# jgrodzki/radix_sort

Hardware: AMD Instinct MI355X
Metric: Gkeys/sec (u64) (higher is better)
Workload: dtype u64

## Files before the change

radix_sort_amd/csrc/rsx_launch_impl.hpp:

```cpp
#pragma once
#include <cstdlib>
#include "rsx_internal.hpp"
#include "rsx_small_kernel.hpp"
#include "rsx_mid_kernels.hpp"
#include "rsx_segment_kernels.hpp"
#include "rsx_segment_pairs_kernels.hpp"

#ifndef RSX_HIST_BLOCKS_PER_CU
#define RSX_HIST_BLOCKS_PER_CU 8
#endif

namespace rsxh {

inline uint32_t rank_atomic_of(const rsx_ctx* ctx) { return (ctx->rank_atomic && !(ctx->options & OPT_BALLOT_RANKS)) ? 1u : 0u; }
constexpr CleanList CLEAN_NONE = {{nullptr, nullptr, nullptr}, {0, 0, 0}};

inline uint64_t hist_blocks_per_region(const rsx_ctx* ctx, const RegionGeom& g) {
    const uint64_t per_block = 512ull * 16;
    uint64_t bpr = ((1ull << g.region_shift) + per_block - 1) / per_block;
    const uint64_t cap = ((uint64_t)ctx->num_cu * RSX_HIST_BLOCKS_PER_CU + g.num_regions - 1) / g.num_regions;
    if (bpr > cap) bpr = cap;
    return bpr == 0 ? 1 : bpr;
}
template <int ES, bool FLT>
// ... 354 lines not shown
    if (grid < parts) grid = parts;
    LaunchTimer lt(ctx, RSX_PROF_HIST, st);
    hipLaunchKernelGGL(rsx_marginal16_kernel<ES>, dim3(grid), dim3(256), 0, st, P, parts, k, g, J, jclear, status32(g) ? 1u : 0u,
                       static_cast<uint4*>(ctx->status), zero16_n, run.clean, run.gate);
    RSX_HIP(hipGetLastError());
    run.clean = CLEAN_NONE;
    return RSX_OK;
}

template <int ES>
int launch_bucket16(rsx_ctx* ctx, const SortRun& run, void* data, void* scratch, size_t n, const rsx_layout* L, const uint64_t* starts,
                    const WidePlan* plan, hipStream_t st) {
    if constexpr (ES < 4) {
        return fail(ctx, RSX_ERR_INTERNAL, "launch_bucket16: narrow elements");
    } else {
        constexpr int KPT = bucket_kpt_for(ES);
        if (L->key_bytes < 4) return fail(ctx, RSX_ERR_INTERNAL, "launch_bucket16: key width out of range");
        SmallArgs a = small_args(ctx, L, L->key_bytes - 2, L->key_bytes, false);
        a.src = data;
        a.data = data;
        a.cap = bucket_cap(ES);
        LaunchTimer lt(ctx, RSX_PROF_OTHER, st);
        const uint64_t avg = (uint64_t)n / 65536u;
        const uint32_t gs = group_shift(ctx, n, L);
        const Gate base = run.gate;
        auto go = [&](auto wgc, auto kc, uint32_t form, uint32_t group_shift) {
            constexpr int WGS = decltype(wgc)::value;
            constexpr int K = decltype(kc)::value;
            SmallArgs b = a;
            b.group_shift = group_shift;
            if (group_shift) b.passes = L->key_bytes;
            static_assert(cape<ES, K, WGS>() == bucket_cape(ES, K, WGS), "host and device agree on what a workgroup holds");
            const size_t lds = (size_t)cape<ES, K, WGS>() * ES + (WGS / 64) * RADIX * bucket_cnt_bytes() + 64 + 3 * RADIX * sizeof(uint32_t);
            auto kern = rsx_bucket16_kernel<ES, K, WGS>;
            ensure_lds(ctx, reinterpret_cast<const void*>(kern), lds);
            int per_cu = (int)((size_t)163840 / lds);
            if (per_cu < 1) per_cu = 1;
            if (per_cu > 4 * RSX_B16_WAVES(WGS) * 64 / WGS) per_cu = 4 * RSX_B16_WAVES(WGS) * 64 / WGS;
            const Gate g{base.word, VERDICT_PATH_MASK | VERDICT_FORM_MASK, VERDICT_HYBRID | form};
            hipLaunchKernelGGL(kern, dim3((uint32_t)(ctx->num_cu * per_cu)), dim3(WGS), lds, st, b, starts, scratch, plan, g);
        };
        using std::integral_constant;
        constexpr int KBIG = wide_kpt_for(ES);
        if (gs >= 2) go(integral_constant<int, 512>{}, integral_constant<int, KPT>{}, VERDICT_GROUPS, gs);
        if (avg <= (uint64_t)256 * KPT) go(integral_constant<int, 256>{}, integral_constant<int, KPT>{}, VERDICT_WG256, 0);
        if (avg <= (uint64_t)512 * KPT) go(integral_constant<int, 512>{}, integral_constant<int, KPT>{}, VERDICT_WG512, 0);
        const bool big_form = KBIG != KPT && wide_big_form(ES, n);
        if (big_form) go(integral_constant<int, 1024>{}, integral_constant<int, KBIG>{}, VERDICT_WG1024, 0);
        else go(integral_constant<int, 1024>{}, integral_constant<int, KPT>{}, VERDICT_WG1024, 0);
        {
            constexpr int KMED = medium_kpt_for(ES);
            const size_t lds = (size_t)cape<ES, KMED, 1024>() * ES + 16 * RADIX * bucket_cnt_bytes() + 64 + 3 * RADIX * sizeof(uint32_t);
            auto kern = rsx_bucket16_medium_kernel<ES, KMED, 1024>;
            ensure_lds(ctx, reinterpret_cast<const void*>(kern), lds);
            const Gate g{base.word, VERDICT_PATH_MASK | VERDICT_MEDIUM, VERDICT_HYBRID | VERDICT_MEDIUM};
            hipLaunchKernelGGL(kern, dim3((uint32_t)ctx->num_cu), dim3(1024), lds, st, a, starts, scratch, plan, (uint32_t)(256 * KPT), (uint32_t)(512 * KPT),
                               (uint32_t)(big_form ? cape<ES, KBIG, 1024>() : cape<ES, KPT, 1024>()), g);
        }
        RSX_HIP(hipGetLastError());
        return RSX_OK;
    }
}

template <int ES>
int launch_segcopy(rsx_ctx* ctx, const void* src, void* dst, const uint64_t* so, const uint64_t* dof,
                   const uint64_t* len, uint32_t nseg, hipStream_t st) {
    const uint32_t bps = 8;
// ... 162 lines not shown
```

radix_sort_amd/csrc/rsx_small_kernel.hpp:

```cpp
#pragma once
#include "rsx_device.hpp"

namespace rsx {

struct SmallArgs {
    const void* src;
    void* data;
    uint32_t n;
    uint32_t passes;
    uint32_t rank_atomic;
    uint32_t map_load;
    uint32_t map_store;
    DigitSpec spec[16];
    KeyXform xf;
    const uint32_t* top_tot;
    uint32_t cap;
    uint32_t no_skip;
    uint32_t group_shift;
    uint32_t key_offset, key_bytes;
    uint32_t* hint;
};

struct PassPlan {
    uint32_t first, end;
    uint32_t mask[8];
    uint32_t low[8];
    __device__ __forceinline__ void set_masks(const uint32_t key_offset, const uint32_t key_bytes) {
#pragma unroll
        for (int w = 0; w < 8; ++w) {
            uint32_t m = 0, l = 0;
#pragma unroll
            for (uint32_t b = 0; b < 4; ++b) {
                const uint32_t byte = 4u * (uint32_t)w + b;
                if (byte >= key_offset + first && byte < key_offset + key_bytes) m |= 0xFFu << (8u * b);
                if (byte >= key_offset && byte < key_offset + first) l |= 0xFFu << (8u * b);
            }
            mask[w] = m;
            low[w] = l;
        }
    }
};

#ifndef RSX_MEND_SLACK
#define RSX_MEND_SLACK 6u
#endif
__device__ __forceinline__ uint32_t first_digit_for(const uint32_t m, const uint32_t variable_bits, const uint32_t end) {
    const uint32_t lg = m <= 1u ? 0u : 32u - (uint32_t)__builtin_clz(m - 1u);
    const uint32_t need = 2u * lg > RSX_MEND_SLACK ? 2u * lg - RSX_MEND_SLACK : 0u;
    uint32_t first = variable_bits > need ? (variable_bits - need) >> 3 : 0u;
    if (first + 1u > end) first = end != 0u ? end - 1u : 0u;
    return first;
}

template <int ES>
struct WaveCnt {
    static constexpr bool HALF = false;
    using T = typename std::conditional<HALF, uint16_t, uint32_t>::type;
    static __device__ __forceinline__ void zero(T* my, uint32_t lane) {
        uint32_t* w = reinterpret_cast<uint32_t*>(my);
#pragma unroll
        for (int i = 0; i < (HALF ? 2 : 4); ++i) w[i * WAVE + lane] = 0;
    }
    static __device__ __forceinline__ uint32_t add_rtn(T* my, uint32_t d, uint32_t v) {
        if constexpr (HALF) {
            const uint32_t sh = (d & 1u) * 16u;
            return (atomicAdd(reinterpret_cast<uint32_t*>(my) + (d >> 1), v << sh) >> sh) & 0xFFFFu;
        } else {
            return atomicAdd(&my[d], v);
        }
    }
};
template <int ES, int KPT, int WG>
__host__ __device__ constexpr uint32_t cape() {
    constexpr uint32_t slots = (uint32_t)WG * KPT;
    constexpr uint32_t room = ((163840u - 1024u - (uint32_t)(WG / WAVE) * RADIX * (uint32_t)sizeof(typename WaveCnt<ES>::T) - 64u - 3u * RADIX * 4u) / (uint32_t)ES) & ~3u;
    return slots < room ? slots : room;
}

template <int ES, int KPT, int WG>
__device__ __forceinline__ void local_load(const SmallArgs& a, const Elem<ES>* __restrict__ src, const uint32_t n, Elem<ES> (&e)[KPT]) {
    const uint32_t tid = threadIdx.x, lane = tid & 63u, wave = tid >> 6;
    const uint32_t kp = (n + WG - 1) / WG;
    const uint32_t seg = wave * (WAVE * kp) + lane;
#pragma unroll
    for (int j = 0; j < KPT; ++j) {
        e[j] = Elem<ES>{};
        if ((uint32_t)j < kp) {
            const uint32_t p = seg + (uint32_t)j * WAVE;
            if (p < n) {
                e[j] = src[p];
                if (a.map_load) key_map<ES, false>(e[j], a.xf);
            }
        }
    }
}

template <int ES, int KPT, int WG>
__device__ __forceinline__ void local_passes(const SmallArgs& a, Elem<ES> (&e)[KPT], const uint32_t n, unsigned char* smem,
                                             const uint32_t first = 0, const uint32_t end = ~0u) {
    const uint32_t stop = end == ~0u ? a.passes : end;
    constexpr int NWAVE = WG / WAVE;
    using E = Elem<ES>;
    E* s_elems = reinterpret_cast<E*>(smem);
    using C = WaveCnt<ES>;
    typename C::T* s_cnt = reinterpret_cast<typename C::T*>(smem + (size_t)cape<ES, KPT, WG>() * sizeof(E));
    uint32_t* s_misc = reinterpret_cast<uint32_t*>(s_cnt + NWAVE * RADIX);
    const uint32_t tid = threadIdx.x, lane = tid & 63u, wave = tid >> 6;
    const uint32_t kp = (n + WG - 1) / WG;
    const uint32_t seg = wave * (WAVE * kp) + lane;
    typename C::T* my = s_cnt + wave * RADIX;
    for (uint32_t pass = first; pass < stop; ++pass) {
        const DigitSpec spec = a.spec[pass];
        C::zero(my, lane);
        auto digit_of = [&](int j) -> uint32_t {
            return (seg + (uint32_t)j * WAVE >= n) ? 255u : elem_digit<ES, false>(e[j], spec);
        };
        uint32_t rk[KPT];
#pragma unroll
        for (int j = 0; j < KPT; ++j) {
            rk[j] = 0;
            if ((uint32_t)j < kp) {
                const uint32_t d = digit_of(j);
                if (a.rank_atomic) {
                    rk[j] = C::add_rtn(my, d, 1u);
                } else {
                    const uint64_t m = match_digit(d);
                    const uint32_t below = mbcnt64(m);
                    const uint32_t seen = my[d];
                    if (below == 0) (void)C::add_rtn(my, d, (uint32_t)__popcll(m));
                    rk[j] = seen + below;
                }
            }
        }
        __syncthreads();
        uint32_t tcount = 0, incl = 0;
        if (tid < RADIX) {
#pragma unroll
            for (int w = 0; w < NWAVE; ++w) tcount += s_cnt[w * RADIX + tid];
            incl = wave_incl_scan<true>(tcount);
            if (lane == 63) s_misc[wave] = incl;
        }
        __syncthreads();
        if (tid < RADIX) {
            uint32_t run = incl - tcount;
            for (uint32_t w = 0; w < wave; ++w) run += s_misc[w];
#pragma unroll
            for (int w = 0; w < NWAVE; ++w) {
                const uint32_t c = s_cnt[w * RADIX + tid];
                s_cnt[w * RADIX + tid] = (typename C::T)run;
                run += c;
            }
        }
        __syncthreads();
#pragma unroll
        for (int j = 0; j < KPT; ++j)
            if ((uint32_t)j < kp) {
                if constexpr (cape<ES, KPT, WG>() < (uint32_t)WG * KPT) {
                    if (seg + (uint32_t)j * WAVE < n) s_elems[(uint32_t)my[digit_of(j)] + rk[j]] = e[j];
                } else {
                    s_elems[(uint32_t)my[digit_of(j)] + rk[j]] = e[j];
                }
            }
        __syncthreads();
        if (pass + 1 < stop) {
#pragma unroll
            for (int j = 0; j < KPT; ++j)
                if ((uint32_t)j < kp) e[j] = s_elems[seg + (uint32_t)j * WAVE];
        }
    }
}

template <int ES, int KPT, int WG>
__device__ __forceinline__ void local_store(const SmallArgs& a, Elem<ES>* __restrict__ dst, const uint32_t n, unsigned char* smem) {
    const Elem<ES>* s_elems = reinterpret_cast<const Elem<ES>*>(smem);
    for (uint32_t i = threadIdx.x; i < n; i += WG) {
        Elem<ES> x = s_elems[i];
        if (a.map_store) key_map<ES, true>(x, a.xf);
        dst[i] = x;
    }
}

template <int ES, int KPT, int WG>
__device__ __forceinline__ void local_sort(const SmallArgs& a, const Elem<ES>* __restrict__ src, Elem<ES>* __restrict__ dst,
                                           const uint32_t n, unsigned char* smem) {
    Elem<ES> e[KPT];
    local_load<ES, KPT, WG>(a, src, n, e);
    local_passes<ES, KPT, WG>(a, e, n, smem);
    local_store<ES, KPT, WG>(a, dst, n, smem);
}

template <int ES, int KPT, int WG, typename DigitFn>
__device__ __forceinline__ void stream_pass(const SmallArgs& a, const Elem<ES>* __restrict__ src, Elem<ES>* __restrict__ dst, const uint32_t m,
                                            unsigned char* smem, DigitFn digit, const bool map_back, uint32_t& bin_start, uint32_t& bin_count) {
    constexpr int NWAVE = WG / WAVE;
    constexpr uint32_t CH = cape<ES, KPT, WG>();
    using E = Elem<ES>;
    E* s_elems = reinterpret_cast<E*>(smem);
    using C = WaveCnt<ES>;
    typename C::T* s_cnt = reinterpret_cast<typename C::T*>(smem + (size_t)cape<ES, KPT, WG>() * sizeof(E));
    uint32_t* s_misc = reinterpret_cast<uint32_t*>(s_cnt + NWAVE * RADIX);
    uint32_t* s_gbase = s_misc + NWAVE;
    uint32_t* s_dstart = s_gbase + RADIX;
// ... 100 lines not shown
    using E = Elem<ES>;
    E* src = buf0;
    E* dst = buf1;
    for (uint32_t pass = 0; pass < a.passes; ++pass) {
        const DigitSpec spec = a.spec[pass];
        uint32_t bs = 0, bc = 0;
        stream_pass<ES, KPT, WG>(a, src, dst, m, smem, [&](const E& x) { return elem_digit<ES, false>(x, spec); },
                                 pass + 1 == a.passes && a.map_store != 0, bs, bc);
        E* t = src;
        src = dst;
        dst = t;
    }
}

#define RSX_B16_WAVES(WG) ((WG) >= 512 ? 4 : 3)
template <int ES>
__device__ __forceinline__ bool agree(const PassPlan& pp, const Elem<ES>& x, const Elem<ES>& y) {
    uint32_t diff = 0;
#pragma unroll
    for (int w = 0; w < ES / 4; ++w) diff |= (x.w[w] ^ y.w[w]) & pp.mask[w];
    return diff == 0;
}
constexpr uint32_t MEND_LIST = 192;
template <int ES, int KPT, int WG>
__device__ __forceinline__ uint32_t* mend_count(unsigned char* smem) {
    return reinterpret_cast<uint32_t*>(smem + (size_t)cape<ES, KPT, WG>() * sizeof(Elem<ES>));
}
template <int ES, int KPT, int WG>
__device__ __forceinline__ bool local_check(const PassPlan& pp, const uint32_t n, unsigned char* smem, Elem<ES> (&x)[KPT], uint32_t& ties) {
    using E = Elem<ES>;
    const E* s_elems = reinterpret_cast<const E*>(smem);
    ties = 0;
    if (threadIdx.x == 0) *mend_count<ES, KPT, WG>(smem) = 0;
#pragma unroll
    for (int j = 0; j < KPT; ++j) {
        const uint32_t i = (uint32_t)j * WG + threadIdx.x;
        x[j] = E{};
        if (i < n) {
            x[j] = s_elems[i];
            const E p = s_elems[i != 0 ? i - 1 : 0];
            uint32_t diff = 0;
#pragma unroll
            for (int w = 0; w < ES / 4; ++w) diff |= (x[j].w[w] ^ p.w[w]) & pp.mask[w];
            ties |= (diff == 0 && i != 0) ? 1u << j : 0u;
        }
    }
    uint32_t work = 0;
    for (uint32_t t = ties; t != 0; t &= t - 1u) {
        const uint32_t i = (uint32_t)__builtin_ctz(t) * WG + threadIdx.x;
        const E u = s_elems[i], v = s_elems[i - 1];
#pragma unroll
        for (int w = 0; w < ES / 4; ++w) work |= (u.w[w] ^ v.w[w]) & pp.low[w];
    }
    return __syncthreads_or(work != 0 ? 1 : 0) != 0;
}
#ifndef RSX_MEND_INLINE
#define RSX_MEND_INLINE __forceinline__
#endif
template <int ES>
struct MendMasks {
    uint32_t hi[ES / 4], lo[ES / 4];
};
template <int ES>
__device__ RSX_MEND_INLINE uint32_t mend_listed(Elem<ES>* s_elems, uint32_t* s_list, uint32_t* s_flag, const uint32_t n, const uint32_t wg,
                                                          uint32_t ties, const MendMasks<ES> mm) {
    using E = Elem<ES>;
    constexpr uint32_t MAX_RUN = 48;
    auto same = [&](const E& u, const E& v) {
        uint32_t diff = 0;
#pragma unroll
        for (int w = 0; w < ES / 4; ++w) diff |= (u.w[w] ^ v.w[w]) & mm.hi[w];
        return diff == 0;
    };
    auto less = [&](const E& u, const E& v) {
#pragma unroll
        for (int w = ES / 4 - 1; w >= 0; --w) {
            const uint32_t a = u.w[w] & mm.lo[w], b = v.w[w] & mm.lo[w];
// ... 16 lines not shown
        const uint32_t i = s_list[1 + threadIdx.x];
        uint32_t len = 2;
        while (i + len < n && len <= MAX_RUN && same(s_elems[i + len], s_elems[i])) ++len;
        if (len > MAX_RUN) {
            *s_flag = 1;
        } else {
            for (uint32_t k = 1; k < len; ++k) {
                const E y = s_elems[i + k];
                uint32_t j = k;
                while (j > 0 && less(y, s_elems[i + j - 1])) {
                    s_elems[i + j] = s_elems[i + j - 1];
                    --j;
                }
                s_elems[i + j] = y;
            }
        }
    }
    __syncthreads();
    return *s_flag == 0 ? 1u : 0u;
}
template <int ES, int KPT, int WG>
__device__ __forceinline__ bool local_mend_listed(const uint32_t n, unsigned char* smem, const PassPlan& pp, uint32_t* s_flag, const uint32_t ties) {
    static_assert((WG / WAVE) * RADIX >= MEND_LIST + 1, "the list lives in the wave counters");
    MendMasks<ES> mm;
#pragma unroll
    for (int w = 0; w < ES / 4; ++w) {
        mm.hi[w] = pp.mask[w];
        mm.lo[w] = pp.low[w];
    }
    return mend_listed<ES>(reinterpret_cast<Elem<ES>*>(smem), mend_count<ES, KPT, WG>(smem), s_flag, n, (uint32_t)WG, ties, mm) != 0;
}
template <int ES, int KPT, int WG>
__device__ __forceinline__ void local_store_regs(const SmallArgs& a, Elem<ES>* __restrict__ dst, const uint32_t n, Elem<ES> (&x)[KPT]) {
#pragma unroll
    for (int j = 0; j < KPT; ++j) {
        const uint32_t i = (uint32_t)j * WG + threadIdx.x;
        if (i < n) {
            if (a.map_store) key_map<ES, true>(x[j], a.xf);
            dst[i] = x[j];
        }
    }
}

template <int ES, int KPT, int WG>
__device__ __forceinline__ bool local_finish(const SmallArgs& a, Elem<ES>* __restrict__ dst, const uint32_t n, unsigned char* smem, const PassPlan& pp,
                                             uint32_t* s_flag) {
    Elem<ES> x[KPT];
    uint32_t ties;
    if (!local_check<ES, KPT, WG>(pp, n, smem, x, ties)) {
        local_store_regs<ES, KPT, WG>(a, dst, n, x);
        return true;
    }
    if (!local_mend_listed<ES, KPT, WG>(n, smem, pp, s_flag, ties)) return false;
    local_store<ES, KPT, WG>(a, dst, n, smem);
    return true;
}

template <int ES, int KPT, int WG>
__device__ __forceinline__ void local_sort_skip(const SmallArgs& a, const Elem<ES>* __restrict__ src, Elem<ES>* __restrict__ dst, const uint32_t n,
                                                unsigned char* smem, PassPlan& pp, uint32_t* s_flag) {
    using E = Elem<ES>;
    E e[KPT];
    local_load<ES, KPT, WG>(a, src, n, e);
    local_passes<ES, KPT, WG>(a, e, n, smem, pp.first, pp.end);
    if (pp.first == 0) {
        local_store<ES, KPT, WG>(a, dst, n, smem);
    } else if (!local_finish<ES, KPT, WG>(a, dst, n, smem, pp, s_flag)) {
        pp.first = 0;
        const uint32_t kp = (n + WG - 1) / WG, seg = (threadIdx.x >> 6) * (WAVE * kp) + (threadIdx.x & 63u);
#pragma unroll
        for (int j = 0; j < KPT; ++j)
            if ((uint32_t)j < kp) e[j] = reinterpret_cast<const E*>(smem)[seg + (uint32_t)j * WAVE];
        __syncthreads();
        local_passes<ES, KPT, WG>(a, e, n, smem, 0, pp.end);
        local_store<ES, KPT, WG>(a, dst, n, smem);
    }
}

template <int ES, int KPT>
__global__ __launch_bounds__(512) void rsx_small_sort_kernel(const SmallArgs a) {
    extern __shared__ __attribute__((aligned(16))) unsigned char smem[];
    local_sort<ES, KPT, 512>(a, static_cast<const Elem<ES>*>(a.src), static_cast<Elem<ES>*>(a.data), a.n, smem);
}

template <int ES, int KPT, int WG>
__global__ __launch_bounds__(WG) void rsx_bucket_sort_kernel(const SmallArgs a) {
    extern __shared__ __attribute__((aligned(16))) unsigned char smem[];
    uint64_t* s_red = reinterpret_cast<uint64_t*>(smem);
    const uint32_t tid = threadIdx.x, v = blockIdx.x;
    uint64_t c = 0;
    if (tid < RADIX) {
        c = a.top_tot[tid];
        if (tid == v) s_red[4] = c;
        if (v == 0) {
            uint64_t big = c;
#pragma unroll
            for (int o = 32; o > 0; o >>= 1) {
                const uint64_t y = __shfl_xor(big, o);
                big = y > big ? y : big;
            }
            if ((tid & 63u) == 0u) s_red[5 + (tid >> 6)] = big;
        }
        uint64_t below = tid < v ? c : 0ull;
#pragma unroll
        for (int o = 32; o > 0; o >>= 1) below += __shfl_xor(below, o);
        if ((tid & 63u) == 0u) s_red[tid >> 6] = below;
    }
    __syncthreads();
    const uint64_t start = s_red[0] + s_red[1] + s_red[2] + s_red[3];
    const uint64_t count = s_red[4];
    if (v == 0 && tid == 0) {
        uint64_t big = s_red[5];
        for (int w = 1; w < 4; ++w) big = s_red[5 + w] > big ? s_red[5 + w] : big;
        __hip_atomic_store(a.hint, big <= (uint64_t)a.cap / 4 ? 1u : big <= (uint64_t)a.cap ? 3u : 2u, __ATOMIC_RELAXED, __HIP_MEMORY_SCOPE_SYSTEM);
    }
    __syncthreads();
    if (count == 0) return;
    if (count > (uint64_t)cape<ES, KPT, WG>()) {
        big_bucket_sort<ES, KPT, WG>(a, const_cast<Elem<ES>*>(static_cast<const Elem<ES>*>(a.src)) + start,
                                     static_cast<Elem<ES>*>(a.data) + start, (uint32_t)count, smem);
        return;
    }
    if constexpr (ES < 8) {
        local_sort<ES, KPT, WG>(a, static_cast<const Elem<ES>*>(a.src) + start, static_cast<Elem<ES>*>(a.data) + start, (uint32_t)count, smem);
    } else {
        PassPlan pp;
        pp.end = a.passes;
        pp.first = a.no_skip ? 0u : first_digit_for((uint32_t)count, 8u * a.passes, a.passes);
        pp.set_masks(a.key_offset, a.key_bytes);
        uint32_t* s_flag = reinterpret_cast<uint32_t*>(reinterpret_cast<typename WaveCnt<ES>::T*>(smem + (size_t)cape<ES, KPT, WG>() * sizeof(Elem<ES>)) + (WG / WAVE) * RADIX) + (WG / WAVE);
        local_sort_skip<ES, KPT, WG>(a, static_cast<const Elem<ES>*>(a.src) + start, static_cast<Elem<ES>*>(a.data) + start, (uint32_t)count, smem, pp,
                                     s_flag);
    }
}

template <int ES, int KPT, int WG>
__global__ __launch_bounds__(WG, RSX_B16_WAVES(WG)) void rsx_bucket16_kernel(const SmallArgs a, const uint64_t* __restrict__ starts, void* scratch,
                                                                         const WidePlan* __restrict__ plan, Gate gate) {
    extern __shared__ __attribute__((aligned(16))) unsigned char smem[];
    if (!gate_open(gate)) return;
    using E = Elem<ES>;
    constexpr int NWAVE = WG / WAVE;
    uint32_t* s_flag = reinterpret_cast<uint32_t*>(reinterpret_cast<typename WaveCnt<ES>::T*>(smem + (size_t)cape<ES, KPT, WG>() * sizeof(E)) + NWAVE * RADIX) + NWAVE;
    const uint32_t gs = a.group_shift != 0 ? plan->group_shift : 0;
    const bool medium = (plan->verdict & VERDICT_MEDIUM) != 0;
    PassPlan pp;
    pp.end = gs == 0 ? plan->pass_end : plan->group_end;
    if (pp.end == 0) {
        if (a.map_store) {
            const uint64_t n = starts[65536];
            E* data = static_cast<E*>(a.data);
            for (uint64_t i = (uint64_t)blockIdx.x * WG + threadIdx.x; i < n; i += (uint64_t)gridDim.x * WG) {
                E x = data[i];
                key_map<ES, true>(x, a.xf);
                data[i] = x;
            }
        }
        return;
    }
    const uint32_t b_lo = plan->window_top - 15u;
    const uint32_t end_sub = pp.end;
    if (gs != 0) pp.end = (b_lo + gs + 7u) / 8u;
    {
        const uint64_t big = (uint64_t)plan->scan_max << gs;
        const uint32_t m = big < (uint64_t)cape<ES, KPT, WG>() ? (uint32_t)big : cape<ES, KPT, WG>();
        pp.first = a.no_skip ? 0u : first_digit_for(m, b_lo + gs, pp.end);
    }
    pp.set_masks(a.key_offset, a.key_bytes);
    for (uint32_t g = blockIdx.x; g < (65536u >> gs); g += gridDim.x) {
        const uint32_t b0 = g << gs;
        const uint64_t gstart = starts[b0];
        const uint64_t gcount = starts[b0 + (1u << gs)] - gstart;
        if (gcount == 0) continue;
        const bool whole = gs == 0 || gcount <= (uint64_t)cape<ES, KPT, WG>();
        const uint32_t nsub = whole ? 1u : 1u << gs;
        for (uint32_t sub = 0; sub < nsub; ++sub) {
            uint64_t start = gstart, count = gcount;
            if (!whole) {
                start = starts[b0 + sub];
                count = starts[b0 + sub + 1] - start;
            }
            if (count != 0) {
                E* bucket = static_cast<E*>(a.data) + start;
                if (count <= (uint64_t)cape<ES, KPT, WG>()) {
                    const uint32_t first = pp.first, end = pp.end;
                    if (!whole) {
                        pp.first = 0;
                        pp.end = end_sub;
                    }
                    local_sort_skip<ES, KPT, WG>(a, bucket, bucket, (uint32_t)count, smem, pp, s_flag);
                    if (!whole) {
                        pp.first = first;
                        pp.end = end;
                    }
                } else if (!medium) {
                    big_bucket_sort<ES, KPT, WG>(a, bucket, static_cast<E*>(scratch) + start, (uint32_t)count, smem);
                }
            }
            __syncthreads();
        }
    }
}

template <int ES, int KPT, int WG>
__global__ __launch_bounds__(WG, RSX_B16_WAVES(WG)) void rsx_bucket16_medium_kernel(const SmallArgs a, const uint64_t* __restrict__ starts, void* scratch,
                                                                                const WidePlan* __restrict__ plan, uint32_t cap256, uint32_t cap512,
                                                                                uint32_t cap1024, Gate gate) {
    extern __shared__ __attribute__((aligned(16))) unsigned char smem[];
    __shared__ uint32_t s_part[2];
    if (!gate_open(gate)) return;
    using E = Elem<ES>;
    constexpr int NWAVE = WG / WAVE;
    constexpr uint32_t CAPE = cape<ES, KPT, WG>();
    uint32_t* s_flag = reinterpret_cast<uint32_t*>(reinterpret_cast<typename WaveCnt<ES>::T*>(smem + (size_t)CAPE * sizeof(E)) + NWAVE * RADIX) + NWAVE;
    const uint32_t tid = threadIdx.x;
    const uint32_t form = plan->verdict & VERDICT_FORM_MASK;
    const uint64_t handled = form == VERDICT_WG256 ? cap256 : form == VERDICT_WG1024 ? cap1024 : cap512;
    const uint32_t end = plan->pass_end;
    if (end == 0) return;
    const uint32_t b_lo = plan->window_top - 15u;
    for (uint32_t b = blockIdx.x; b < 65536u; b += gridDim.x) {
        const uint64_t start = starts[b];
        const uint64_t count = starts[b + 1] - start;
        if (count <= handled) continue;
        E* bucket = static_cast<E*>(a.data) + start;
        E* scr = static_cast<E*>(scratch) + start;
// ... 49 lines not shown
```

radix_sort_amd/csrc/rsx_segment_pairs_kernels.hpp:

```cpp
#pragma once
#include "rsx_pairs_kernels.hpp"
#include "rsx_segment_kernels.hpp"

namespace rsx {

struct SegPairsArgs {
    uint8_t* keys;
    uint8_t* values;
    void* w0;
    void* w1;
    uint64_t n;
    const uint64_t* offsets;
    uint64_t nseg;
    uint64_t row_len;
    uint64_t lo, hi;
    uint32_t team;
    uint32_t* error;
    uint32_t kind, desc, mode, ib;
};

template <int ES, int KB, int VB>
__device__ __forceinline__ Elem<ES> segp_join(const SegPairsArgs& s, const uint64_t beg, const uint32_t p) {
    static_assert(pairs_elem(KB, VB) == (uint32_t)ES, "the joined element of these widths");
    constexpr int VOFF = (int)pairs_voff(KB, VB);
// ... 30 lines not shown
    using K = typename PairsKey<KB>::type;
    unsigned char r[ES];
    __builtin_memcpy(r, &x, ES);
    if (s.mode != SEGP_LOCAL) {
        K k;
        __builtin_memcpy(&k, r, KB);
        reinterpret_cast<K*>(s.keys)[beg + i] = pairs_unmap<K>(k, s.kind, s.desc);
    }
    if constexpr (VB > 0) {
        using V = typename PairsWord<VB>::type;
        bool column = true;
        if constexpr (VB == 4) {
            if (s.mode != SEGP_VALUES) {
                uint32_t pos;
                __builtin_memcpy(&pos, r + VOFF, 4);
                if (s.mode == SEGP_GLOBAL) *reinterpret_cast<uint32_t*>(s.values + (beg + i) * ES + VOFF) = pos;
                else if (s.ib == 8) reinterpret_cast<uint64_t*>(s.values)[beg + i] = pos;
                else reinterpret_cast<uint32_t*>(s.values)[beg + i] = pos;
                column = false;
            }
        }
        if (column) {
            V v;
            __builtin_memcpy(&v, r + VOFF, VB);
            reinterpret_cast<V*>(s.values)[beg + i] = v;
        }
    }
}

template <int ES, int KPT, int WG>
__device__ __forceinline__ void segp_passes_skip(const SmallArgs& a, Elem<ES> (&e)[KPT], const uint32_t n, unsigned char* smem, PassPlan& pp,
                                                 uint32_t* s_flag) {
    using E = Elem<ES>;
    local_passes<ES, KPT, WG>(a, e, n, smem, pp.first, pp.end);
    if (pp.first == 0) return;
    uint32_t ties;
    bool mended;
    {
        E x[KPT];
        mended = !local_check<ES, KPT, WG>(pp, n, smem, x, ties);
    }
    if (!mended) mended = local_mend_listed<ES, KPT, WG>(n, smem, pp, s_flag, ties);
    if (!mended) {
        pp.first = 0;
        const uint32_t kp = (n + WG - 1) / WG, seg = (threadIdx.x >> 6) * (WAVE * kp) + (threadIdx.x & 63u);
#pragma unroll
        for (int j = 0; j < KPT; ++j)
            if ((uint32_t)j < kp) e[j] = reinterpret_cast<const E*>(smem)[seg + (uint32_t)j * WAVE];
        __syncthreads();
        local_passes<ES, KPT, WG>(a, e, n, smem, 0, pp.end);
    }
}

template <int ES, int KB, int VB, int KPT, int WG, bool MEM>
__device__ __forceinline__ void segp_sort_one(const SmallArgs& a, const SegPairsArgs& s, const uint64_t beg, const uint32_t len, unsigned char* smem,
                                              uint32_t& skip_ok) {
    using E = Elem<ES>;
    if constexpr (MEM) {
        E* src = static_cast<E*>(s.w0) + beg;
        E* dst = static_cast<E*>(s.w1) + beg;
        for (uint32_t i = threadIdx.x; i < len; i += WG) src[i] = segp_join<ES, KB, VB>(s, beg, i);
        __builtin_amdgcn_fence(__ATOMIC_RELEASE, "agent");
        __syncthreads();
        __builtin_amdgcn_fence(__ATOMIC_ACQUIRE, "agent");
        for (uint32_t pass = 0; pass < a.passes; ++pass) {
            const DigitSpec spec = a.spec[pass];
            uint32_t bs = 0, bc = 0;
            stream_pass<ES, KPT, WG>(a, src, dst, len, smem, [&](const E& x) { return elem_digit<ES, false>(x, spec); }, false, bs, bc);
            E* t = src;
            src = dst;
            dst = t;
        }
        for (uint32_t i = threadIdx.x; i < len; i += WG) segp_split<ES, KB, VB>(s, beg, i, src[i]);
    } else {
        E e[KPT];
        {
            const uint32_t lane = threadIdx.x & 63u, wave = threadIdx.x >> 6;
            const uint32_t kp = (len + WG - 1) / WG;
            const uint32_t seg = wave * (WAVE * kp) + lane;
#pragma unroll
            for (int j = 0; j < KPT; ++j) {
                e[j] = E{};
                if ((uint32_t)j < kp) {
// ... 80 lines not shown
```

Baseline: 67.93.

## Use wider 11-bit digits for in-LDS bucket sort of 64-bit keys

Adds a wide-digit local radix pass path for 8-byte elements in the 16-bit bucket kernel. It uses 11-bit digits with atomic ranking, phased counter sets and vectorised scans, so fewer LDS passes are needed per bucket. The bit-level skip logic chooses a starting bit instead of a starting byte, and the masks are rebuilt at bit granularity. This trades fewer passes for larger counter arrays laid over the tile, extra barriers from the rank phases, and more complex scans. The path is only taken when atomic ranking is enabled.

```diff
diff --git a/radix_sort_amd/csrc/rsx_launch_impl.hpp b/radix_sort_amd/csrc/rsx_launch_impl.hpp
--- a/radix_sort_amd/csrc/rsx_launch_impl.hpp
+++ b/radix_sort_amd/csrc/rsx_launch_impl.hpp
@@ -410,7 +410,10 @@
             if (group_shift) b.passes = L->key_bytes;
             static_assert(cape<ES, K, WGS>() == bucket_cape(ES, K, WGS), "host and device agree on what a workgroup holds");
             const size_t lds = (size_t)cape<ES, K, WGS>() * ES + (WGS / 64) * RADIX * bucket_cnt_bytes() + 64 + 3 * RADIX * sizeof(uint32_t);
-            auto kern = rsx_bucket16_kernel<ES, K, WGS>;
+            auto kern = rsx_bucket16_kernel<ES, K, WGS, 8>;
+            if constexpr (ES == 8 && RSX_B16_DIGIT_BITS != 8) {
+                if (b.rank_atomic) kern = rsx_bucket16_kernel<ES, K, WGS, RSX_B16_DIGIT_BITS>;
+            }
             ensure_lds(ctx, reinterpret_cast<const void*>(kern), lds);
             int per_cu = (int)((size_t)163840 / lds);
             if (per_cu < 1) per_cu = 1;
diff --git a/radix_sort_amd/csrc/rsx_small_kernel.hpp b/radix_sort_amd/csrc/rsx_small_kernel.hpp
--- a/radix_sort_amd/csrc/rsx_small_kernel.hpp
+++ b/radix_sort_amd/csrc/rsx_small_kernel.hpp
@@ -37,6 +37,19 @@
             }
             mask[w] = m;
             low[w] = l;
+        }
+    }
+    uint32_t wfrom, wtop;
+    __device__ __forceinline__ void set_masks_at_bit(const uint32_t key_offset, const uint32_t key_bytes) {
+        const uint32_t kb0 = 8u * key_offset, kb1 = 8u * (key_offset + key_bytes), split = kb0 + wfrom;
+        auto below = [](const uint32_t bit, const uint32_t w) -> uint32_t {
+            return bit <= 32u * w ? 0u : bit >= 32u * w + 32u ? ~0u : (1u << (bit - 32u * w)) - 1u;
+        };
+#pragma unroll
+        for (int w = 0; w < 8; ++w) {
+            const uint32_t key = below(kb1, (uint32_t)w) & ~below(kb0, (uint32_t)w), lo = below(split, (uint32_t)w);
+            mask[w] = key & ~lo;
+            low[w] = key & lo;
         }
     }
 };
@@ -168,6 +181,134 @@
                 if ((uint32_t)j < kp) e[j] = s_elems[seg + (uint32_t)j * WAVE];
         }
     }
+}
+
+#ifndef RSX_B16_DIGIT_BITS
+#define RSX_B16_DIGIT_BITS 11
+#endif
+#ifndef RSX_B16_RANK_PHASES
+#define RSX_B16_RANK_PHASES 2
+#endif
+#ifndef RSX_B16_RANK_PHASES_512
+#define RSX_B16_RANK_PHASES_512 1
+#endif
+#ifndef RSX_MEND_SLACK_WIDE
+#define RSX_MEND_SLACK_WIDE 8u
+#endif
+template <int DB>
+__device__ __forceinline__ uint32_t first_bit_for(const uint32_t m, const uint32_t variable_bits) {
+    const uint32_t lg = m <= 1u ? 0u : 32u - (uint32_t)__builtin_clz(m - 1u);
+    const uint32_t need = 2u * lg > RSX_MEND_SLACK_WIDE ? 2u * lg - RSX_MEND_SLACK_WIDE : 0u;
+    const uint32_t cover = (uint32_t)DB * (need == 0u ? 1u : (need + (uint32_t)DB - 1u) / (uint32_t)DB);
+    return variable_bits > cover ? variable_bits - cover : 0u;
+}
+
+template <int KPT, int WG, int DB>
+__device__ __forceinline__ void local_passes_wide(const SmallArgs& a, Elem<8> (&e)[KPT], const uint32_t n, unsigned char* smem, const uint32_t from,
+                                                  const uint32_t top) {
+    using E = Elem<8>;
+    constexpr int NWAVE = WG / WAVE;
+    constexpr int DPT = (1 << DB) / WG;
+    constexpr int PHW = WG == 512 ? RSX_B16_RANK_PHASES_512 : RSX_B16_RANK_PHASES;
+    constexpr int PH = PHW < NWAVE ? PHW : NWAVE;
+    constexpr int NSET = NWAVE / PH;
+    static_assert(PH >= 1 && (PH & (PH - 1)) == 0 && NSET * PH == NWAVE, "phases: a power of two");
+    static_assert(DPT == 2 || DPT == 4 || DPT == 8, "the scan reads 2, 4 or 8 consecutive counters per thread");
+    static_assert(cape<8, KPT, WG>() == (uint32_t)WG * KPT, "padding slots are scattered too: LDS has all WG * KPT slots");
+    static_assert((size_t)NWAVE * (1u << DB) * sizeof(uint32_t) <= (size_t)WG * KPT * sizeof(E), "the counters lie over the tile");
+    constexpr int VEC = DPT < 4 ? DPT : 4;
+    typedef uint32_t cvec __attribute__((ext_vector_type(VEC)));
+    constexpr int NV = DPT / VEC;
+    E* s_elems = reinterpret_cast<E*>(smem);
+    uint32_t* s_cnt = reinterpret_cast<uint32_t*>(smem);
+    uint32_t* s_misc = reinterpret_cast<uint32_t*>(smem + (size_t)cape<8, KPT, WG>() * sizeof(E));
+    const uint32_t tid = threadIdx.x, lane = tid & 63u, wave = tid >> 6;
+    const uint32_t kp = (n + WG - 1) / WG;
+    const uint32_t seg = wave * (WAVE * kp) + lane;
+    uint32_t pos = from;
+    do {
+        const uint32_t width = top > pos ? (top - pos < (uint32_t)DB ? top - pos : (uint32_t)DB) : 1u;
+        const bool last = pos + width >= top;
+        const uint32_t sh = 8u * a.key_offset + pos, dmask = (1u << width) - 1u;
+        const uint32_t nd = 1u << (width < 3u ? 3u : width);
+        uint32_t* my = s_cnt + (wave / PH) * nd;
+        if ((uint32_t)__builtin_amdgcn_readfirstlane((int)wave) % PH == 0)
+            for (uint32_t i = lane; i < nd / 4u; i += WAVE) reinterpret_cast<uint4*>(my)[i] = make_uint4(0, 0, 0, 0);
+        auto digit_of = [&](int j) -> uint32_t {
+            const uint64_t k = ((uint64_t)e[j].w[1] << 32) | e[j].w[0];
+            return (seg + (uint32_t)j * WAVE >= n) ? dmask : (uint32_t)(k >> sh) & dmask;
+        };
+        const uint32_t turn = (uint32_t)__builtin_amdgcn_readfirstlane((int)wave) % PH;
+        for (uint32_t i = 0; i < turn; ++i) __syncthreads();
+        uint32_t rk[KPT];
+#pragma unroll
+        for (int j = 0; j < KPT; ++j) {
+            rk[j] = 0;
+            if ((uint32_t)j < kp) rk[j] = atomicAdd(&my[digit_of(j)], 1u);
+        }
+        for (uint32_t i = turn; i < (uint32_t)PH; ++i) __syncthreads();
+        const bool scans = tid * DPT < nd;
+        const uint32_t* col = s_cnt + tid * DPT;
+        uint32_t tot[DPT];
+#pragma unroll
+        for (int k = 0; k < DPT; ++k) tot[k] = 0;
+        if (scans) {
+#pragma unroll
+            for (int w = 0; w < NSET; ++w)
+#pragma unroll
+                for (int v = 0; v < NV; ++v) {
+                    const cvec c = reinterpret_cast<const cvec*>(col + (uint32_t)w * nd)[v];
+#pragma unroll
+                    for (int k = 0; k < DPT / NV; ++k) tot[v * (DPT / NV) + k] += c[k];
+                }
+        }
+        uint32_t mine = 0;
+#pragma unroll
+        for (int k = 0; k < DPT; ++k) mine += tot[k];
+        const uint32_t incl = wave_incl_scan<true>(mine);
+        if (lane == 63) s_misc[wave] = incl;
+        __syncthreads();
+        if (scans) {
+            uint32_t run = incl - mine;
+            for (uint32_t w = 0; w < wave; ++w) run += s_misc[w];
+#pragma unroll
+            for (int k = 0; k < DPT; ++k) {
+                const uint32_t c = tot[k];
+                tot[k] = run;
+                run += c;
+            }
+#pragma unroll
+            for (int w = 0; w < NSET; ++w)
+#pragma unroll
+                for (int v = 0; v < NV; ++v) {
+                    cvec* p = reinterpret_cast<cvec*>(const_cast<uint32_t*>(col) + (uint32_t)w * nd) + v;
+                    const cvec c = *p;
+                    cvec b;
+#pragma unroll
+                    for (int k = 0; k < DPT / NV; ++k) {
+                        b[k] = tot[v * (DPT / NV) + k];
+                        tot[v * (DPT / NV) + k] += c[k];
+                    }
+                    *p = b;
+                }
+        }
+        __syncthreads();
+#pragma unroll
+        for (int j = 0; j < KPT; ++j)
+            if ((uint32_t)j < kp) rk[j] += my[digit_of(j)];
+        __syncthreads();
+#pragma unroll
+        for (int j = 0; j < KPT; ++j)
+            if ((uint32_t)j < kp) s_elems[rk[j]] = e[j];
+        __syncthreads();
+        if (!last) {
+#pragma unroll
+            for (int j = 0; j < KPT; ++j)
+                if ((uint32_t)j < kp) e[j] = s_elems[seg + (uint32_t)j * WAVE];
+            __syncthreads();
+        }
+        pos += width;
+    } while (pos < top);
 }
 
 template <int ES, int KPT, int WG>
@@ -451,23 +592,29 @@
     return true;
 }
 
-template <int ES, int KPT, int WG>
+template <int ES, int KPT, int WG, int DB = 8>
 __device__ __forceinline__ void local_sort_skip(const SmallArgs& a, const Elem<ES>* __restrict__ src, Elem<ES>* __restrict__ dst, const uint32_t n,
                                                 unsigned char* smem, PassPlan& pp, uint32_t* s_flag) {
     using E = Elem<ES>;
+    static_assert(DB == 8 || ES == 8, "wide digits: 8-byte elements");
     E e[KPT];
     local_load<ES, KPT, WG>(a, src, n, e);
-    local_passes<ES, KPT, WG>(a, e, n, smem, pp.first, pp.end);
+    if constexpr (DB == 8) local_passes<ES, KPT, WG>(a, e, n, smem, pp.first, pp.end);
+    else local_passes_wide<KPT, WG, DB>(a, e, n, smem, pp.wfrom, pp.wtop);
     if (pp.first == 0) {
         local_store<ES, KPT, WG>(a, dst, n, smem);
     } else if (!local_finish<ES, KPT, WG>(a, dst, n, smem, pp, s_flag)) {
         pp.first = 0;
+        pp.wfrom = 0;
         const uint32_t kp = (n + WG - 1) / WG, seg = (threadIdx.x >> 6) * (WAVE * kp) + (threadIdx.x & 63u);
 #pragma unroll
-        for (int j = 0; j < KPT; ++j)
+        for (int j = 0; j < KPT; ++j) {
+            if constexpr (DB != 8) e[j] = E{};
             if ((uint32_t)j < kp) e[j] = reinterpret_cast<const E*>(smem)[seg + (uint32_t)j * WAVE];
-        __syncthreads();
-        local_passes<ES, KPT, WG>(a, e, n, smem, 0, pp.end);
+        }
+        __syncthreads();
+        if constexpr (DB == 8) local_passes<ES, KPT, WG>(a, e, n, smem, 0, pp.end);
+        else local_passes_wide<KPT, WG, DB>(a, e, n, smem, 0, pp.wtop);
         local_store<ES, KPT, WG>(a, dst, n, smem);
     }
 }
@@ -529,7 +676,7 @@
     }
 }
 
-template <int ES, int KPT, int WG>
+template <int ES, int KPT, int WG, int DB = 8>
 __global__ __launch_bounds__(WG, RSX_B16_WAVES(WG)) void rsx_bucket16_kernel(const SmallArgs a, const uint64_t* __restrict__ starts, void* scratch,
                                                                          const WidePlan* __restrict__ plan, Gate gate) {
     extern __shared__ __attribute__((aligned(16))) unsigned char smem[];
@@ -560,8 +707,15 @@
         const uint64_t big = (uint64_t)plan->scan_max << gs;
         const uint32_t m = big < (uint64_t)cape<ES, KPT, WG>() ? (uint32_t)big : cape<ES, KPT, WG>();
         pp.first = a.no_skip ? 0u : first_digit_for(m, b_lo + gs, pp.end);
-    }
-    pp.set_masks(a.key_offset, a.key_bytes);
+        pp.wtop = b_lo + gs;
+        pp.wfrom = a.no_skip ? 0u : first_bit_for<DB>(m, b_lo + gs);
+    }
+    if constexpr (DB == 8) {
+        pp.set_masks(a.key_offset, a.key_bytes);
+    } else {
+        pp.first = pp.wfrom != 0u ? 1u : 0u;
+        pp.set_masks_at_bit(a.key_offset, a.key_bytes);
+    }
     for (uint32_t g = blockIdx.x; g < (65536u >> gs); g += gridDim.x) {
         const uint32_t b0 = g << gs;
         const uint64_t gstart = starts[b0];
@@ -578,15 +732,19 @@
             if (count != 0) {
                 E* bucket = static_cast<E*>(a.data) + start;
                 if (count <= (uint64_t)cape<ES, KPT, WG>()) {
-                    const uint32_t first = pp.first, end = pp.end;
+                    const uint32_t first = pp.first, end = pp.end, wfrom = pp.wfrom, wtop = pp.wtop;
                     if (!whole) {
                         pp.first = 0;
                         pp.end = end_sub;
+                        pp.wfrom = 0;
+                        pp.wtop = b_lo;
                     }
-                    local_sort_skip<ES, KPT, WG>(a, bucket, bucket, (uint32_t)count, smem, pp, s_flag);
+                    local_sort_skip<ES, KPT, WG, DB>(a, bucket, bucket, (uint32_t)count, smem, pp, s_flag);
                     if (!whole) {
                         pp.first = first;
                         pp.end = end;
+                        pp.wfrom = wfrom;
+                        pp.wtop = wtop;
                     }
                 } else if (!medium) {
                     big_bucket_sort<ES, KPT, WG>(a, bucket, static_cast<E*>(scratch) + start, (uint32_t)count, smem);
```

Result: slower. 66.64 (-1.9%).

## Batch LDS and global accesses in groups to expose memory-level parallelism in local sort

Applied to the files above, without the earlier changes.

Restructures the local sort's load, ranking, scatter, check and store loops to issue groups of independent LDS and global accesses before consuming them. Bounds checks are hoisted per group, and out-of-range global loads are clamped so the loads stay unconditional. Wave index is made uniform via readfirstlane, and the fallback re-sort paths are folded into loops so local_passes is instantiated once instead of twice. The aim is more memory-level parallelism and smaller code, at the cost of higher register pressure and some redundant clamped loads.

```diff
diff --git a/radix_sort_amd/csrc/rsx_segment_pairs_kernels.hpp b/radix_sort_amd/csrc/rsx_segment_pairs_kernels.hpp
--- a/radix_sort_amd/csrc/rsx_segment_pairs_kernels.hpp
+++ b/radix_sort_amd/csrc/rsx_segment_pairs_kernels.hpp
@@ -86,23 +86,25 @@
 __device__ __forceinline__ void segp_passes_skip(const SmallArgs& a, Elem<ES> (&e)[KPT], const uint32_t n, unsigned char* smem, PassPlan& pp,
                                                  uint32_t* s_flag) {
     using E = Elem<ES>;
-    local_passes<ES, KPT, WG>(a, e, n, smem, pp.first, pp.end);
-    if (pp.first == 0) return;
-    uint32_t ties;
-    bool mended;
-    {
-        E x[KPT];
-        mended = !local_check<ES, KPT, WG>(pp, n, smem, x, ties);
-    }
-    if (!mended) mended = local_mend_listed<ES, KPT, WG>(n, smem, pp, s_flag, ties);
-    if (!mended) {
+    for (;;) {
+        local_passes<ES, KPT, WG>(a, e, n, smem, pp.first, pp.end);
+        if (pp.first == 0) return;
+        uint32_t ties;
+        bool mended;
+        {
+            E x[KPT];
+            mended = !local_check<ES, KPT, WG>(pp, n, smem, x, ties);
+        }
+        if (!mended) mended = local_mend_listed<ES, KPT, WG>(n, smem, pp, s_flag, ties);
+        if (mended) return;
         pp.first = 0;
         const uint32_t kp = (n + WG - 1) / WG, seg = (threadIdx.x >> 6) * (WAVE * kp) + (threadIdx.x & 63u);
 #pragma unroll
-        for (int j = 0; j < KPT; ++j)
+        for (int j = 0; j < KPT; ++j) {
+            e[j] = E{};
             if ((uint32_t)j < kp) e[j] = reinterpret_cast<const E*>(smem)[seg + (uint32_t)j * WAVE];
+        }
         __syncthreads();
-        local_passes<ES, KPT, WG>(a, e, n, smem, 0, pp.end);
     }
 }
 
diff --git a/radix_sort_amd/csrc/rsx_small_kernel.hpp b/radix_sort_amd/csrc/rsx_small_kernel.hpp
--- a/radix_sort_amd/csrc/rsx_small_kernel.hpp
+++ b/radix_sort_amd/csrc/rsx_small_kernel.hpp
@@ -77,21 +77,52 @@
     return slots < room ? slots : room;
 }
 
+#ifndef RSX_LDS_GROUP
+#define RSX_LDS_GROUP 4
+#endif
+template <int KPT>
+__host__ __device__ constexpr int lds_group() {
+    return KPT > 5 * RSX_LDS_GROUP ? (KPT + 1) / 2 : RSX_LDS_GROUP;
+}
+
+constexpr int WAITCNT_VMCNT0 = (7 << 4) | (15 << 8);
+static_assert(WAITCNT_VMCNT0 == 0x0F70, "s_waitcnt vmcnt(0)");
+
+__device__ __forceinline__ uint32_t here(uint32_t v) {
+    asm volatile("" : "+v"(v));
+    return v;
+}
+
 template <int ES, int KPT, int WG>
 __device__ __forceinline__ void local_load(const SmallArgs& a, const Elem<ES>* __restrict__ src, const uint32_t n, Elem<ES> (&e)[KPT]) {
+    constexpr int G = lds_group<KPT>();
     const uint32_t tid = threadIdx.x, lane = tid & 63u, wave = tid >> 6;
     const uint32_t kp = (n + WG - 1) / WG;
     const uint32_t seg = wave * (WAVE * kp) + lane;
 #pragma unroll
-    for (int j = 0; j < KPT; ++j) {
-        e[j] = Elem<ES>{};
-        if ((uint32_t)j < kp) {
-            const uint32_t p = seg + (uint32_t)j * WAVE;
-            if (p < n) {
-                e[j] = src[p];
-                if (a.map_load) key_map<ES, false>(e[j], a.xf);
-            }
-        }
+    for (int j0 = 0; j0 < KPT; j0 += G) {
+#pragma unroll
+        for (int j = j0; j < j0 + G && j < KPT; ++j) e[j] = Elem<ES>{};
+        const int JE = j0 + G < KPT ? j0 + G : KPT;
+        if ((uint32_t)JE <= kp) {
+#pragma unroll
+            for (int j = j0; j < JE; ++j) {
+                const uint32_t p = seg + (uint32_t)j * WAVE;
+                e[j] = src[p < n ? p : n - 1u];
+            }
+        } else if ((uint32_t)j0 < kp) {
+#pragma unroll
+            for (int j = j0; j < JE; ++j)
+                if ((uint32_t)j < kp) {
+                    const uint32_t p = seg + (uint32_t)j * WAVE;
+                    e[j] = src[p < n ? p : n - 1u];
+                }
+        }
+    }
+    if (a.map_load) {
+#pragma unroll
+        for (int j = 0; j < KPT; ++j)
+            if ((uint32_t)j < kp) key_map<ES, false>(e[j], a.xf);
     }
 }
 
@@ -105,10 +136,15 @@
     using C = WaveCnt<ES>;
     typename C::T* s_cnt = reinterpret_cast<typename C::T*>(smem + (size_t)cape<ES, KPT, WG>() * sizeof(E));
     uint32_t* s_misc = reinterpret_cast<uint32_t*>(s_cnt + NWAVE * RADIX);
-    const uint32_t tid = threadIdx.x, lane = tid & 63u, wave = tid >> 6;
+    const uint32_t tid = threadIdx.x, lane = tid & 63u;
+    const uint32_t wave = (uint32_t)__builtin_amdgcn_readfirstlane((int)(tid >> 6));
     const uint32_t kp = (n + WG - 1) / WG;
     const uint32_t seg = wave * (WAVE * kp) + lane;
     typename C::T* my = s_cnt + wave * RADIX;
+    constexpr int G = lds_group<KPT>();
+    constexpr bool ALL_SLOTS = cape<ES, KPT, WG>() >= (uint32_t)WG * KPT;
+    const uint32_t wave_end = (wave + 1u) * (WAVE * kp);
+    const uint32_t write_end = (ALL_SLOTS || wave_end < n) ? wave_end : n;
     for (uint32_t pass = first; pass < stop; ++pass) {
         const DigitSpec spec = a.spec[pass];
         C::zero(my, lane);
@@ -116,14 +152,27 @@
             return (seg + (uint32_t)j * WAVE >= n) ? 255u : elem_digit<ES, false>(e[j], spec);
         };
         uint32_t rk[KPT];
-#pragma unroll
-        for (int j = 0; j < KPT; ++j) {
-            rk[j] = 0;
-            if ((uint32_t)j < kp) {
-                const uint32_t d = digit_of(j);
-                if (a.rank_atomic) {
-                    rk[j] = C::add_rtn(my, d, 1u);
-                } else {
+        if (a.rank_atomic) {
+#pragma unroll
+            for (int j0 = 0; j0 < KPT; j0 += G) {
+                const int JE = j0 + G < KPT ? j0 + G : KPT;
+#pragma unroll
+                for (int j = j0; j < JE; ++j) rk[j] = 0;
+                if ((uint32_t)JE <= kp) {
+#pragma unroll
+                    for (int j = j0; j < JE; ++j) rk[j] = C::add_rtn(my, digit_of(j), 1u);
+                } else if ((uint32_t)j0 < kp) {
+#pragma unroll
+                    for (int j = j0; j < JE; ++j)
+                        if ((uint32_t)j < kp) rk[j] = C::add_rtn(my, digit_of(j), 1u);
+                }
+            }
+        } else {
+#pragma unroll
+            for (int j = 0; j < KPT; ++j) {
+                rk[j] = 0;
+                if ((uint32_t)j < kp) {
+                    const uint32_t d = digit_of(j);
                     const uint64_t m = match_digit(d);
                     const uint32_t below = mbcnt64(m);
                     const uint32_t seen = my[d];
@@ -133,34 +182,60 @@
             }
         }
         __syncthreads();
-        uint32_t tcount = 0, incl = 0;
-        if (tid < RADIX) {
-#pragma unroll
-            for (int w = 0; w < NWAVE; ++w) tcount += s_cnt[w * RADIX + tid];
-            incl = wave_incl_scan<true>(tcount);
-            if (lane == 63) s_misc[wave] = incl;
-        }
-        __syncthreads();
-        if (tid < RADIX) {
-            uint32_t run = incl - tcount;
-            for (uint32_t w = 0; w < wave; ++w) run += s_misc[w];
-#pragma unroll
-            for (int w = 0; w < NWAVE; ++w) {
-                const uint32_t c = s_cnt[w * RADIX + tid];
-                s_cnt[w * RADIX + tid] = (typename C::T)run;
-                run += c;
-            }
-        }
-        __syncthreads();
-#pragma unroll
-        for (int j = 0; j < KPT; ++j)
-            if ((uint32_t)j < kp) {
-                if constexpr (cape<ES, KPT, WG>() < (uint32_t)WG * KPT) {
-                    if (seg + (uint32_t)j * WAVE < n) s_elems[(uint32_t)my[digit_of(j)] + rk[j]] = e[j];
+        {
+            uint32_t tcount = 0, incl = 0;
+            if (tid < RADIX) {
+#pragma unroll
+                for (int w0 = 0; w0 < NWAVE; w0 += G) {
+                    uint32_t c[G];
+#pragma unroll
+                    for (int w = w0; w < w0 + G && w < NWAVE; ++w) c[w - w0] = s_cnt[w * RADIX + tid];
+#pragma unroll
+                    for (int w = w0; w < w0 + G && w < NWAVE; ++w) tcount += c[w - w0];
+                }
+                incl = wave_incl_scan<true>(tcount);
+                if (lane == 63) s_misc[wave] = incl;
+            }
+            __syncthreads();
+            if (tid < RADIX) {
+                uint32_t run = incl - tcount;
+                for (uint32_t w = 0; w < wave; ++w) run += s_misc[w];
+#pragma unroll
+                for (int w0 = 0; w0 < NWAVE; w0 += G) {
+                    uint32_t c[G];
+#pragma unroll
+                    for (int w = w0; w < w0 + G && w < NWAVE; ++w) c[w - w0] = s_cnt[w * RADIX + tid];
+#pragma unroll
+                    for (int w = w0; w < w0 + G && w < NWAVE; ++w) {
+                        s_cnt[w * RADIX + tid] = (typename C::T)run;
+                        run += c[w - w0];
+                    }
+                }
+            }
+            __syncthreads();
+        }
+#pragma unroll
+        for (int j0 = 0; j0 < KPT; j0 += G) {
+            const int JE = j0 + G < KPT ? j0 + G : KPT;
+            if ((uint32_t)JE <= kp) {
+#pragma unroll
+                for (int j = j0; j < JE; ++j) rk[j] += (uint32_t)my[digit_of(j)];
+                if constexpr (ALL_SLOTS) {
+#pragma unroll
+                    for (int j = j0; j < JE; ++j) s_elems[rk[j]] = e[j];
                 } else {
-                    s_elems[(uint32_t)my[digit_of(j)] + rk[j]] = e[j];
-                }
-            }
+#pragma unroll
+                    for (int j = j0; j < JE; ++j)
+                        if (seg + (uint32_t)j * WAVE < write_end) s_elems[rk[j]] = e[j];
+                }
+            } else if ((uint32_t)j0 < kp) {
+#pragma unroll
+                for (int j = j0; j < JE; ++j)
+                    if ((uint32_t)j < kp) {
+                        if (ALL_SLOTS || seg + (uint32_t)j * WAVE < write_end) s_elems[(uint32_t)my[digit_of(j)] + rk[j]] = e[j];
+                    }
+            }
+        }
         __syncthreads();
         if (pass + 1 < stop) {
 #pragma unroll
@@ -168,6 +243,7 @@
                 if ((uint32_t)j < kp) e[j] = s_elems[seg + (uint32_t)j * WAVE];
         }
     }
+    __builtin_amdgcn_s_waitcnt(WAITCNT_VMCNT0);
 }
 
 template <int ES, int KPT, int WG>
@@ -334,17 +410,35 @@
     const E* s_elems = reinterpret_cast<const E*>(smem);
     ties = 0;
     if (threadIdx.x == 0) *mend_count<ES, KPT, WG>(smem) = 0;
-#pragma unroll
-    for (int j = 0; j < KPT; ++j) {
-        const uint32_t i = (uint32_t)j * WG + threadIdx.x;
-        x[j] = E{};
-        if (i < n) {
-            x[j] = s_elems[i];
-            const E p = s_elems[i != 0 ? i - 1 : 0];
-            uint32_t diff = 0;
-#pragma unroll
-            for (int w = 0; w < ES / 4; ++w) diff |= (x[j].w[w] ^ p.w[w]) & pp.mask[w];
-            ties |= (diff == 0 && i != 0) ? 1u << j : 0u;
+    constexpr int G = lds_group<KPT>();
+    const uint32_t tid = here(threadIdx.x);
+    const uint32_t last = n != 0 ? n - 1u : 0u;
+#pragma unroll
+    for (int j0 = 0; j0 < KPT; j0 += G) {
+#pragma unroll
+        for (int j = j0; j < j0 + G && j < KPT; ++j) x[j] = E{};
+        if ((uint32_t)j0 * WG < n) {
+            E p[G];
+#pragma unroll
+            for (int j = j0; j < j0 + G && j < KPT; ++j) {
+                const uint32_t i = (uint32_t)j * WG + tid, ii = i < last ? i : last;
+                if (j == 0) {
+                    x[j] = s_elems[ii];
+                    p[j - j0] = s_elems[ii != 0 ? ii - 1u : 0u];
+                } else {
+                    const uint32_t pi = (ii != 0 ? ii : 1u) - 1u;
+                    p[j - j0] = s_elems[pi];
+                    x[j] = s_elems[pi + 1u];
+                }
+            }
+#pragma unroll
+            for (int j = j0; j < j0 + G && j < KPT; ++j) {
+                const uint32_t i = (uint32_t)j * WG + tid;
+                uint32_t diff = 0;
+#pragma unroll
+                for (int w = 0; w < ES / 4; ++w) diff |= (x[j].w[w] ^ p[j - j0].w[w]) & pp.mask[w];
+                ties |= (diff == 0 && i != 0 && i < n) ? 1u << j : 0u;
+            }
         }
     }
     uint32_t work = 0;
@@ -427,12 +521,28 @@
 }
 template <int ES, int KPT, int WG>
 __device__ __forceinline__ void local_store_regs(const SmallArgs& a, Elem<ES>* __restrict__ dst, const uint32_t n, Elem<ES> (&x)[KPT]) {
-#pragma unroll
-    for (int j = 0; j < KPT; ++j) {
-        const uint32_t i = (uint32_t)j * WG + threadIdx.x;
-        if (i < n) {
-            if (a.map_store) key_map<ES, true>(x[j], a.xf);
-            dst[i] = x[j];
+    constexpr int G = lds_group<KPT>();
+    const uint32_t tid = here(threadIdx.x);
+    if (a.map_store) {
+#pragma unroll
+        for (int j0 = 0; j0 < KPT; j0 += G)
+            if ((uint32_t)j0 * WG < n) {
+#pragma unroll
+                for (int j = j0; j < j0 + G && j < KPT; ++j) key_map<ES, true>(x[j], a.xf);
+            }
+    }
+#pragma unroll
+    for (int j0 = 0; j0 < KPT; j0 += G) {
+        const int JE = j0 + G < KPT ? j0 + G : KPT;
+        if ((uint32_t)JE * WG <= n) {
+#pragma unroll
+            for (int j = j0; j < JE; ++j) dst[(uint32_t)j * WG + tid] = x[j];
+        } else if ((uint32_t)j0 * WG < n) {
+#pragma unroll
+            for (int j = j0; j < JE; ++j) {
+                const uint32_t i = (uint32_t)j * WG + tid;
+                if (i < n) dst[i] = x[j];
+            }
         }
     }
 }
@@ -457,18 +567,21 @@
     using E = Elem<ES>;
     E e[KPT];
     local_load<ES, KPT, WG>(a, src, n, e);
-    local_passes<ES, KPT, WG>(a, e, n, smem, pp.first, pp.end);
-    if (pp.first == 0) {
-        local_store<ES, KPT, WG>(a, dst, n, smem);
-    } else if (!local_finish<ES, KPT, WG>(a, dst, n, smem, pp, s_flag)) {
+    for (;;) {
+        local_passes<ES, KPT, WG>(a, e, n, smem, pp.first, pp.end);
+        if (pp.first == 0) {
+            local_store<ES, KPT, WG>(a, dst, n, smem);
+            break;
+        }
+        if (local_finish<ES, KPT, WG>(a, dst, n, smem, pp, s_flag)) break;
         pp.first = 0;
         const uint32_t kp = (n + WG - 1) / WG, seg = (threadIdx.x >> 6) * (WAVE * kp) + (threadIdx.x & 63u);
 #pragma unroll
-        for (int j = 0; j < KPT; ++j)
+        for (int j = 0; j < KPT; ++j) {
+            e[j] = E{};
             if ((uint32_t)j < kp) e[j] = reinterpret_cast<const E*>(smem)[seg + (uint32_t)j * WAVE];
-        __syncthreads();
-        local_passes<ES, KPT, WG>(a, e, n, smem, 0, pp.end);
-        local_store<ES, KPT, WG>(a, dst, n, smem);
+        }
+        __syncthreads();
     }
 }
 
```

After: 67.97 before, 69.90 after (median of 6 runs). 2.8% higher.
